# alex-petrenko/sample-factory

Hardware: AMD Instinct MI355X
Metric: env-steps/sec (whole node), 4096 envs, 84x84x4 obs (higher is better)
Workload: dtype f32

## Files before the change

### sample_factory_amd/csrc/sf_nn_img.h

```cpp
#pragma once

#ifndef SF_IMG_FLIP
#define SF_IMG_FLIP 1
#endif
#ifndef SF_IMG_PRIO
#define SF_IMG_PRIO 0
#endif
#ifndef SF_IMG_HALFSTEP
#define SF_IMG_HALFSTEP 1
#endif
template <int CIN, int H, int W, int KS, int ST, int TMF, int WSETS, int R>
struct ImgFwdGeom {
    static constexpr int OH = (H - KS) / ST + 1, OW = (W - KS) / ST + 1, OHW = R * OW;
    static constexpr int U = OH / R, HU = (R - 1) * ST + KS;
    static constexpr int K = KS * KS * CIN, KG = K / 16;
    static constexpr int C4 = CIN / 4, WQ = W / ST;
    static constexpr int PLANE_USED = ST * HU * WQ;
    static constexpr int PLANE = SF_IMG_FLIP ? (PLANE_USED + 15) / 16 * 16 : PLANE_USED;
    static constexpr int IMG_CH = C4 * PLANE;
    static constexpr int IMG_B = (IMG_CH * 16 + 1023) / 1024 * 1024;
    static constexpr int BROWS = WSETS * TMF * 16;
    static constexpr int RING = (2 * BROWS - 2) / OHW + 2;
    static_assert(CIN % 16 == 0 && W % ST == 0 && K % 16 == 0 && OH % R == 0, "geometry");
    static_assert(RING * IMG_B <= 160 * 1024, "LDS");
};

template <int CIN, int H, int W, int KS, int ST, int TMF, int WSETS, int R>
__global__ __launch_bounds__(256 * WSETS, 1) void k_fwd_img(const float *__restrict__ in, int64_t in_stride,
                                                    const float *__restrict__ wt, const float *__restrict__ bias,
                                                    float *__restrict__ out, int nsamples, int act) {
    typedef ImgFwdGeom<CIN, H, W, KS, ST, TMF, WSETS, R> G;
    constexpr int NW = 4 * WSETS, TB = TMF * WSETS;
    constexpr int OW = G::OW, OHW = G::OHW, K = G::K, KG = G::KG, WQ = G::WQ, PLANE = G::PLANE, RING = G::RING;
    constexpr int IMG_B = G::IMG_B, N = 64, U = G::U, HU = G::HU;
    __shared__ __attribute__((aligned(1024))) char ring[RING * IMG_B];
    const int tid = threadIdx.x, lane = tid & 63, wave = __builtin_amdgcn_readfirstlane(tid >> 6);
    const int col = lane & 15, kg = lane >> 4, n = (wave & 3) * 16 + col, wset = wave >> 2;
#if SF_IMG_PRIO
    if (__builtin_amdgcn_s_getreg((3 << 11) | (0 << 6) | 4) & 1u) __builtin_amdgcn_s_setprio(SF_IMG_PRIO);
#endif
    const int nunits = nsamples * U;
    const int64_t Mtot = (int64_t)nunits * OHW;
    const int total_frags = (int)((Mtot + 15) >> 4);
    const int per = (total_frags + (int)gridDim.x - 1) / (int)gridDim.x;
    const int f_beg = (int)blockIdx.x * per, f_end = min(total_frags, f_beg + per);
    if (f_beg >= f_end) return;
    f32x4 breg[KG];
#pragma unroll
    for (int g = 0; g < KG; ++g)
        breg[g] = *reinterpret_cast<const f32x4 *>(__builtin_assume_aligned(wt + (int64_t)n * K + 16 * g + 4 * kg, 16));
    const float bv = bias ? bias[n] : 0.f;

    constexpr int NDMA = IMG_B / 1024, NI = (NDMA + NW - 1) / NW;
    int srcoff[NI];
#pragma unroll
    for (int j = 0; j < NI; ++j) {
        int q = (wave + NW * j) * 64 + lane;
        q = q < G::IMG_CH ? q : 0;
        const int c = q / PLANE;
        int r0 = q - c * PLANE;
        r0 = r0 < G::PLANE_USED ? r0 : 0;
        const int pw = r0 / (HU * WQ), r1 = r0 - pw * (HU * WQ);
        const int ihl = r1 / WQ, iwq = r1 - ihl * WQ;
        const int ih = SF_IMG_FLIP ? HU - 1 - ihl : ihl;
        srcoff[j] = (ih * W + iwq * ST + pw) * CIN + c * 4;
    }
    auto load_image = [&](int s) {
        const int u = s < nunits ? s : nunits - 1, smp = u / U, strip = u - smp * U;
        const float *img = in + (int64_t)smp * in_stride + strip * (R * ST * W * CIN);
        char *dst = ring + (s % RING) * IMG_B;
#pragma unroll
        for (int j = 0; j < NI; ++j)
            if (wave + NW * j < NDMA) GLDS16(img + srcoff[j], dst + (wave + NW * j) * 1024);
    };
    const uint32_t M32 = (uint32_t)Mtot;
    auto last_sample = [&](int fb, int nf) {
        uint32_t m = (uint32_t)(fb + nf) * 16u - 1u;
        m = m < M32 ? m : M32 - 1u;
        return (int)(m / (uint32_t)OHW);
    };
    int loaded = (int)(((uint32_t)f_beg * 16u) / (uint32_t)OHW);
    {
        const int hi = last_sample(f_beg, min(TB, f_end - f_beg));
        for (; loaded <= hi; ++loaded) load_image(loaded);
    }
    f32x4 pend[TMF];
    int pend_fb = -1, pend_nf = 0;
    auto store_pend = [&]() {
        float *ob = out + ((int64_t)pend_fb * 16 + 4 * kg) * N + n;
        const int rows_left = (int)(M32 - ((uint32_t)pend_fb * 16u + 4u * (uint32_t)kg));
#pragma unroll
        for (int f = 0; f < TMF; ++f)
#pragma unroll
            for (int r = 0; r < 4; ++r)
                if (f < pend_nf && f * 16 + r < rows_left) ob[(f * 16 + r) * N] = pend[f][r];
    };
    for (int fb0 = f_beg; fb0 < f_end; fb0 += TB) {
        const int fb = fb0 + wset * TMF;
        const int nf = max(0, min(TMF, f_end - fb));
        asm volatile("s_waitcnt vmcnt(0)" ::: "memory");
        __syncthreads();
        if (fb0 + TB < f_end) {
            const int hi = last_sample(fb0 + TB, min(TB, f_end - fb0 - TB));
            for (; loaded <= hi; ++loaded) load_image(loaded);
        }
        if (pend_fb >= 0) store_pend();
        int base[TMF];
#pragma unroll
        for (int f = 0; f < TMF; ++f) {
            uint32_t m = (uint32_t)(nf > 0 ? fb + (f < nf ? f : 0) : fb0) * 16u + (uint32_t)col;
            m = m < M32 ? m : M32 - 1u;
            const uint32_t s = m / (uint32_t)OHW, p = m - s * (uint32_t)OHW, oh = p / (uint32_t)OW, ow = p - oh * (uint32_t)OW;
            const uint32_t prow = SF_IMG_FLIP ? ((uint32_t)(R - 1) - oh) * ST : oh * ST;
            base[f] = (int)((s % (uint32_t)RING) * (uint32_t)IMG_B + ((uint32_t)kg * PLANE + prow * WQ + ow) * 16u);
        }
        auto compute = [&](auto nfc) {
        constexpr int NF = decltype(nfc)::value;
        f32x4 acc[NF];
#pragma unroll
        for (int f = 0; f < NF; ++f) acc[f] = f32x4{0.f, 0.f, 0.f, 0.f};
        static_assert(KG % 2 == 0, "k-groups come in pairs");
        f32x4 a[2][2][NF];
        auto fetch = [&](int g, int slot) {
            const int tap = (16 * g) / CIN, cb = ((16 * g) % CIN) / 4, kh = tap / KS, kw = tap % KS;
            const int imm = (cb * PLANE + ((kw % ST) * HU + (SF_IMG_FLIP ? KS - 1 - kh : kh)) * WQ + kw / ST) * 16;
#pragma unroll
            for (int f = 0; f < NF; ++f)
                a[slot][g & 1][f] = *reinterpret_cast<const f32x4 *>(__builtin_assume_aligned(ring + base[f] + imm, 16));
        };
        auto mfmas = [&](int g, int slot) {
#pragma unroll
            for (int j = 0; j < 4; ++j)
#pragma unroll
                for (int f = 0; f < NF; ++f)
                    acc[f] = __builtin_amdgcn_mfma_f32_16x16x4f32(a[slot][g & 1][f][j], breg[g][j], acc[f], 0, 0, 0);
        };
        fetch(0, 0);
        fetch(1, 0);
#pragma unroll
        for (int gp = 0; gp < KG / 2; ++gp) {
            mfmas(2 * gp, gp & 1);
            __builtin_amdgcn_sched_barrier(0);
            if (gp + 1 < KG / 2) {
                fetch(2 * gp + 2, (gp + 1) & 1);
                fetch(2 * gp + 3, (gp + 1) & 1);
            }
            __builtin_amdgcn_sched_barrier(0);
            mfmas(2 * gp + 1, gp & 1);
            __builtin_amdgcn_sched_barrier(0);
        }
        auto park = [&](auto kc) {
            constexpr int KIND = decltype(kc)::value;
#pragma unroll
            for (int f = 0; f < NF; ++f)
#pragma unroll
                for (int r = 0; r < 4; ++r) pend[f][r] = act_fwd_c<KIND>(acc[f][r] + bv, act);
        };
        if (act == 1) park(std::integral_constant<int, 1>{});
        else park(std::integral_constant<int, -1>{});
        };
        if (SF_IMG_HALFSTEP && TMF == 2 && nf == 1) compute(std::integral_constant<int, 1>{});
        else compute(std::integral_constant<int, TMF>{});
        pend_fb = fb;
        pend_nf = nf;
    }
    if (pend_fb >= 0) store_pend();
}
```

### sample_factory_amd/csrc/sf_nn_glds.h

```cpp
#pragma once

#ifndef SF_GLDS_ABLATE
#define SF_GLDS_ABLATE 0
#endif
#define GLDS16(gsrc, ldst)                                                                       \
    __builtin_amdgcn_global_load_lds((const __attribute__((address_space(1))) void *)(gsrc),    \
                                     (__attribute__((address_space(3))) void *)(ldst), 16, 0, 0)

#define BARRIER_NOFENCE()                  \
    do {                                   \
        asm volatile("" ::: "memory");     \
        __builtin_amdgcn_s_barrier();      \
        asm volatile("" ::: "memory");     \
    } while (0)

template <int TM, int TN>
__device__ __forceinline__ void mma_chunk_rows(const float *__restrict__ As, const float *__restrict__ Bs, int arow0,
                                               int brow0, int lane, f32x16 (&acc)[TM][TN]) {
    const int r = lane & 31, h = lane >> 5, sw = (r >> 1) & 7;
    const float *ap = As + (arow0 + r) * 32, *bp = Bs + (brow0 + r) * 32;
#pragma unroll
    for (int c = 0; c < 4; ++c) {
        const int pos = (((2 * c + h) ^ sw) << 2);
        float4 a[TM], b[TN];
// ... 36 lines not shown
                    j == 0 ? b[c & 1][tn].x : j == 1 ? b[c & 1][tn].y : j == 2 ? b[c & 1][tn].z : b[c & 1][tn].w,
                    acc[tm][tn], 0, 0, 0);
    };
    fetch(0);
#pragma unroll
    for (int c = 0; c < 4; ++c) {
        mfmas(c, 0);
        mfmas(c, 1);
        __builtin_amdgcn_sched_barrier(0);
        mid(c);
        if (c + 1 < 4) fetch(c + 1);
        __builtin_amdgcn_sched_barrier(0);
        mfmas(c, 2);
        mfmas(c, 3);
    }
}

__device__ __forceinline__ void glds16_s(const void *ubase, uint32_t voff, uint32_t lds_byte_addr) {
    asm volatile("s_mov_b32 m0, %0\n\ts_nop 0\n\tglobal_load_lds_dwordx4 %1, %2"
                 :: "s"(lds_byte_addr), "v"(voff), "s"(ubase) : "memory", "m0");
}

template <int I, int N, typename F>
__device__ __forceinline__ void sf_static_for(F &&f) {
    if constexpr (I < N) {
        f(std::integral_constant<int, I>{});
        sf_static_for<I + 1, N>(f);
    }
}
template <int IMM>
__device__ __forceinline__ void glds16_si(const void *ubase, uint32_t voff, uint32_t lds_base) {
    asm volatile("s_add_u32 m0, %0, %3\n\ts_nop 0\n\tglobal_load_lds_dwordx4 %1, %2"
                 :: "s"(lds_base), "v"(voff), "s"(ubase), "n"(IMM) : "memory", "m0", "scc");
}

template <int TM, int TN, int OFF, typename F>
__device__ __forceinline__ void mma_chunk_ptrs_mid(const float *const (&ap)[4], const float *const (&bp)[4],
                                                   f32x16 (&acc)[TM][TN], F &&mid) {
    float4 a[2][TM], b[2][TN];
    auto fetch = [&](int c) {
#pragma unroll
        for (int i = 0; i < TM; ++i) a[c & 1][i] = *reinterpret_cast<const float4 *>(ap[c] + OFF + i * 32 * 32);
#pragma unroll
        for (int i = 0; i < TN; ++i) b[c & 1][i] = *reinterpret_cast<const float4 *>(bp[c] + OFF + i * 32 * 32);
    };
    auto mfmas = [&](int c, int j) {
#pragma unroll
        for (int tm = 0; tm < TM; ++tm)
#pragma unroll
            for (int tn = 0; tn < TN; ++tn)
                acc[tm][tn] = __builtin_amdgcn_mfma_f32_32x32x2f32(
                    j == 0 ? a[c & 1][tm].x : j == 1 ? a[c & 1][tm].y : j == 2 ? a[c & 1][tm].z : a[c & 1][tm].w,
                    j == 0 ? b[c & 1][tn].x : j == 1 ? b[c & 1][tn].y : j == 2 ? b[c & 1][tn].z : b[c & 1][tn].w,
                    acc[tm][tn], 0, 0, 0);
    };
    fetch(0);
#pragma unroll
    for (int c = 0; c < 4; ++c) {
        mfmas(c, 0);
        mfmas(c, 1);
        __builtin_amdgcn_sched_barrier(0);
        mid(c);
        if (c + 1 < 4) fetch(c + 1);
        __builtin_amdgcn_sched_barrier(0);
        mfmas(c, 2);
        mfmas(c, 3);
    }
}

template <int TM, int TN, int OFF, bool ZEROC = false>
__device__ __forceinline__ void mma_chunk_ptrs(const float *const (&ap)[4], const float *const (&bp)[4],
                                               f32x16 (&acc)[TM][TN]) {
#pragma unroll
    for (int c = 0; c < 4; ++c) {
        float4 a[TM], b[TN];
#pragma unroll
        for (int i = 0; i < TM; ++i) a[i] = *reinterpret_cast<const float4 *>(ap[c] + OFF + i * 32 * 32);
#pragma unroll
        for (int i = 0; i < TN; ++i) b[i] = *reinterpret_cast<const float4 *>(bp[c] + OFF + i * 32 * 32);
#pragma unroll
        for (int j = 0; j < 4; ++j)
#pragma unroll
            for (int tm = 0; tm < TM; ++tm)
#pragma unroll
                for (int tn = 0; tn < TN; ++tn) {
                    const f32x16 zero = {0.f, 0.f, 0.f, 0.f, 0.f, 0.f, 0.f, 0.f, 0.f, 0.f, 0.f, 0.f, 0.f, 0.f, 0.f, 0.f};
                    acc[tm][tn] = __builtin_amdgcn_mfma_f32_32x32x2f32(
                        j == 0 ? a[tm].x : j == 1 ? a[tm].y : j == 2 ? a[tm].z : a[tm].w,
                        j == 0 ? b[tn].x : j == 1 ? b[tn].y : j == 2 ? b[tn].z : b[tn].w,
                        (ZEROC && c == 0 && j == 0) ? zero : acc[tm][tn], 0, 0, 0);
                }
    }
}

#ifndef SF_FWD_FRAG_DB
#define SF_FWD_FRAG_DB 0
#endif
#ifndef SF_QUADROW_FRAG_DB
#define SF_QUADROW_FRAG_DB 2
#endif
template <int P> using HookPt = std::integral_constant<int, P>;
#ifndef SF_FRAG_DB_SINK
#define SF_FRAG_DB_SINK 16
#endif
template <int TM, int TN, int OFF, bool ZEROC = false, bool SPREAD = false, typename F>
__device__ __forceinline__ void mma_chunk_ptrs_db(const float *const (&ap)[4], const float *const (&bp)[4],
                                                  f32x16 (&acc)[TM][TN], F &&hook) {
    float4 a[2][TM], b[2][TN];
    auto fetch = [&](int c) {
#pragma unroll
        for (int i = 0; i < TM; ++i) a[c & 1][i] = *reinterpret_cast<const float4 *>(ap[c] + OFF + i * 32 * 32);
#pragma unroll
        for (int i = 0; i < TN; ++i) b[c & 1][i] = *reinterpret_cast<const float4 *>(bp[c] + OFF + i * 32 * 32);
    };
    auto mfmas = [&](int c, int j) {
#pragma unroll
        for (int tm = 0; tm < TM; ++tm)
#pragma unroll
            for (int tn = 0; tn < TN; ++tn) {
                const f32x16 zero = {0.f, 0.f, 0.f, 0.f, 0.f, 0.f, 0.f, 0.f, 0.f, 0.f, 0.f, 0.f, 0.f, 0.f, 0.f, 0.f};
                acc[tm][tn] = __builtin_amdgcn_mfma_f32_32x32x2f32(
                    j == 0 ? a[c & 1][tm].x : j == 1 ? a[c & 1][tm].y : j == 2 ? a[c & 1][tm].z : a[c & 1][tm].w,
                    j == 0 ? b[c & 1][tn].x : j == 1 ? b[c & 1][tn].y : j == 2 ? b[c & 1][tn].z : b[c & 1][tn].w,
                    (ZEROC && c == 0 && j == 0) ? zero : acc[tm][tn], 0, 0, 0);
            }
    };
    constexpr int PER = TM * TN;
    fetch(0);
    hook(HookPt<0>{});
#pragma unroll
    for (int c = 0; c < 4; ++c) {
        mfmas(c, 0);
        if (c + 1 < 4 || c == 0) {
            __builtin_amdgcn_sched_barrier(0);
            if (c == 0) hook(HookPt<1>{});
            if (c + 1 < 4) fetch(c + 1);
            __builtin_amdgcn_sched_barrier(0);
        } else if (SF_FRAG_DB_SINK == 3 * PER) __builtin_amdgcn_sched_barrier(0);
        mfmas(c, 1);
        if (c == 0 && SPREAD) {
            __builtin_amdgcn_sched_barrier(0);
            hook(HookPt<2>{});
            __builtin_amdgcn_sched_barrier(0);
        }
        if (c == 3 && SF_FRAG_DB_SINK == 2 * PER) __builtin_amdgcn_sched_barrier(0);
        mfmas(c, 2);
        if (c == 3 && SF_FRAG_DB_SINK == PER) __builtin_amdgcn_sched_barrier(0);
        mfmas(c, 3);
        if (c == 0) hook(HookPt<3>{});
        if (c == 3 && SF_FRAG_DB_SINK == 0) __builtin_amdgcn_sched_barrier(0);
    }
}

#ifndef SF_PIX_INCR
#define SF_PIX_INCR 1
#endif
#ifndef SF_PIX_LDSIMM
#define SF_PIX_LDSIMM 1
#endif
#ifndef SF_QUADROW_ROT
#define SF_QUADROW_ROT 0
#endif
#ifndef SF_QUADROW_PREP
#define SF_QUADROW_PREP 1
#endif
#ifndef SF_DGRAD_PIX_ZL_LITE
#define SF_DGRAD_PIX_ZL_LITE 1
#endif
template <int TM, int TN, int STAGE_F>
__device__ __forceinline__ void mma_chunk_stage(const float *const (&ap)[4], const float *const (&bp)[4], int stage,
                                                f32x16 (&acc)[TM][TN]) {
    if (stage == 0) mma_chunk_ptrs<TM, TN, 0>(ap, bp, acc);
    else mma_chunk_ptrs<TM, TN, STAGE_F>(ap, bp, acc);
}

template <int BM, int BN, int WM, int WN, int NS, bool ZL, bool PERSIST = false, bool DYNLDS = false>
__device__ __forceinline__ void fwd_glds_body(ConvG g, const float *__restrict__ in, int64_t in_stride,
                                              const float *__restrict__ wt, const float *__restrict__ bias,
                                              float *__restrict__ out, int64_t Mtot, int k_per_split,
                                              float *__restrict__ partial, const float *__restrict__ dmask,
                                              int dmask_on, int rx, int ry, int rtot, int tap_perm, int bx_shift = 0) {
    constexpr int TM = BM / WM / 32, TN = BN / WN / 32;
    constexpr int AI = BM / 32, BI = BN / 32;
    constexpr int STAGE = (BM + BN) * 32;
    static_assert(WM * WN == 4 && TM >= 1 && TN >= 1 && (NS == 2 || NS == 3), "4 waves per block");
    __shared__ __attribute__((aligned(1024))) float lds_static[DYNLDS ? 1 : NS * STAGE];
    extern __shared__ __attribute__((aligned(1024))) float lds_dynamic[];
    float *const lds = DYNLDS ? lds_dynamic : lds_static;
    const int tid = threadIdx.x, lane = tid & 63, wave = __builtin_amdgcn_readfirstlane(tid >> 6);
    const int wm = wave / WN, wn = wave % WN;
    const int ptiles = PERSIST ? (int)((Mtot + BM - 1) / BM) : 1;
    for (int ptile = PERSIST ? (int)blockIdx.x : 0; ptile < ptiles; ptile += PERSIST ? (int)gridDim.x : 1) {
    int bx = PERSIST ? ptile : (int)blockIdx.x + bx_shift, by = blockIdx.y, bz = blockIdx.z;
    if (rtot > 0) {
        const int per = (rtot + 7) >> 3, L = (int)(blockIdx.x & 7u) * per + (int)(blockIdx.x >> 3);
        if (L >= rtot) return;
        by = L % ry;
        const int t = L / ry;
        bx = t % rx;
        bz = t / rx;
    }
    const int64_t m0 = (int64_t)bx * BM;
    const int n0 = by * BN;
    const int N = g.Cout, K = g.K;
    const int kbeg = bz * k_per_split, kend = min(K, kbeg + k_per_split);

    const int lrow = lane >> 3, lpos = lane & 7;
    const float *asrc[AI], *bsrc[BI];
#pragma unroll
    for (int i = 0; i < AI; ++i) {
        const int row = (i * 4 + wave) * 8 + lrow;
        int64_t m = m0 + row;
        m = m < Mtot ? m : Mtot - 1;
        const uint32_t smp = fdiv((uint32_t)m, g.dOHOW), pix = (uint32_t)m - smp * (uint32_t)(g.OH * g.OW);
        asrc[i] = in + (int64_t)smp * in_stride + patch_origin<false>(g, pix) + ((lpos ^ ((row >> 1) & 7)) << 2);
    }
#pragma unroll
    for (int i = 0; i < BI; ++i) {
        const int row = (i * 4 + wave) * 8 + lrow;
        int n = n0 + row;
        n = n < N ? n : N - 1;
        bsrc[i] = wt + (int64_t)n * K + ((lpos ^ ((row >> 1) & 7)) << 2);
    }
    f32x16 acc[TM][TN];
#pragma unroll
    for (int a_ = 0; a_ < TM; ++a_)
#pragma unroll
        for (int b_ = 0; b_ < TN; ++b_)
#pragma unroll
            for (int r_ = 0; r_ < 16; ++r_) acc[a_][b_][r_] = 0.f;

    auto issue = [&](int k0, int stage) {
        const uint32_t tap = fdiv((uint32_t)k0, g.dCin), c0 = (uint32_t)k0 - tap * (uint32_t)g.Cin;
        const uint32_t kh = fdiv(tap, g.dKW), kw = tap - kh * (uint32_t)g.KW;
        const int aoff = (int)((kh * (uint32_t)g.W + kw) * (uint32_t)g.Cin + c0);
        float *sa = lds + stage * STAGE, *sb = sa + BM * 32;
#pragma unroll
        for (int i = 0; i < AI; ++i) GLDS16(asrc[i] + aoff, sa + (i * 4 + wave) * 256);
#pragma unroll
        for (int i = 0; i < BI; ++i) GLDS16(bsrc[i] + k0, sb + (i * 4 + wave) * 256);
    };
    static_assert(NS == 2, "two LDS stages");
    const bool tapperm = tap_perm && g.KH == 4 && g.KW == 4 && g.S == 2 && g.Cin == 32 && kbeg == 0 && kend == K;
    auto kord = [&](int k0) {
        if (!tapperm) return k0;
        const int p = k0 >> 5, grp = p >> 2, e = p & 3;
        const int kh = ((grp >> 1) & 1) + 2 * (e >> 1), kw = (grp & 1) + 2 * (e & 1);
        return (kh * 4 + kw) << 5;
    };
    int stage = 0, k0 = kbeg;
    constexpr bool MASK_PRE = ZL && TM * TN == 4;
    float mpre[MASK_PRE ? TM : 1][MASK_PRE ? TN : 1][16];
    bool mask_pre = false;
    auto prefetch_mask = [&]() {
        if constexpr (MASK_PRE) {
            if (dmask_on && dmask && g.relu == 1 && m0 + BM <= Mtot && n0 + BN <= N) {
                const float *mk = dmask + (m0 + wm * TM * 32) * N + (n0 + wn * TN * 32);
                const uint32_t vo = (uint32_t)(4 * (lane >> 5)) * (uint32_t)N + (uint32_t)(lane & 31);
#pragma unroll
                for (int tm = 0; tm < TM; ++tm)
#pragma unroll
                    for (int tn = 0; tn < TN; ++tn)
#pragma unroll
                        for (int r = 0; r < 16; ++r)
                            mpre[tm][tn][r] = (mk + (int64_t)(tm * 32 + (r & 3) + 8 * (r >> 2)) * N + tn * 32)[vo];
                mask_pre = true;
            }
        }
    };
    if constexpr (ZL) {

        uint32_t avoff[AI], bvoff[BI];
#pragma unroll
        for (int i = 0; i < AI; ++i) avoff[i] = (uint32_t)((asrc[i] - in) * (int64_t)sizeof(float));
#pragma unroll
        for (int i = 0; i < BI; ++i) bvoff[i] = (uint32_t)((bsrc[i] - wt) * (int64_t)sizeof(float));
        const uint32_t lds0 = (uint32_t)(uintptr_t)(__attribute__((address_space(3))) float *)lds;
        const int r = lane & 31, h = lane >> 5, sw = (r >> 1) & 7;
        const float *apl[4], *bpl[4];
#pragma unroll
        for (int c = 0; c < 4; ++c) {
            const int pos = (((2 * c + h) ^ sw) << 2);
            apl[c] = lds + (wm * TM * 32 + r) * 32 + pos;
            bpl[c] = lds + BM * 32 + (wn * TN * 32 + r) * 32 + pos;
        }
        auto chunk_off = [&](int kn) {
            const uint32_t tap = fdiv((uint32_t)kn, g.dCin), c0 = (uint32_t)kn - tap * (uint32_t)g.Cin;
            const uint32_t kh = fdiv(tap, g.dKW), kw = tap - kh * (uint32_t)g.KW;
            return (int)((kh * (uint32_t)g.W + kw) * (uint32_t)g.Cin + c0);
        };
        auto dma = [&](int q, const float *abase, const float *bbase, int st) {
            if (q < AI) glds16_s(abase, avoff[q < AI ? q : 0], lds0 + (uint32_t)((st * STAGE + (q * 4 + wave) * 256) * 4));
            else glds16_s(bbase, bvoff[q >= AI ? q - AI : 0], lds0 + (uint32_t)((st * STAGE + BM * 32 + ((q - AI) * 4 + wave) * 256) * 4));
        };
        {
            const int kf = kord(kbeg);
            const float *ab = in + chunk_off(kf), *bb = wt + kf;
#pragma unroll
            for (int q = 0; q < AI + BI; ++q) dma(q, ab, bb, 0);
        }
        auto step = [&](auto stc, bool prefetch) {
            constexpr int ST = decltype(stc)::value;
            asm volatile("s_waitcnt vmcnt(0)" ::: "memory");
            BARRIER_NOFENCE();
            const int kn = prefetch ? kord(k0 + 32) : 0;
            const float *ab = in + chunk_off(kn), *bb = wt + kn;
            if (!prefetch) prefetch_mask();
            if constexpr (TM * TN <= 2) {
                mma_chunk_ptrs_mid<TM, TN, ST * STAGE>(apl, bpl, acc, [&](int c) {
                    constexpr int TOT = AI + BI, PER = (TOT + 2) / 3;
                    if (prefetch) {
#pragma unroll
                        for (int q = 0; q < TOT; ++q)
                            if (q / PER == c) dma(q, ab, bb, ST ^ 1);
                    }
                });
            } else {
                auto burst = [&](int qlo, int qhi) {
                    if (prefetch) {
#pragma unroll
                        for (int q = 0; q < AI + BI; ++q)
                            if (q >= qlo && q < qhi) dma(q, ab, bb, ST ^ 1);
                    }
                };
                if constexpr (SF_FWD_FRAG_DB >= 2) {
                    mma_chunk_ptrs_db<TM, TN, ST * STAGE, false, SF_FWD_FRAG_DB == 3>(apl, bpl, acc, [&](auto pt) {
                        constexpr int P = decltype(pt)::value, HALF = (AI + BI) / 2;
                        if constexpr (SF_FWD_FRAG_DB == 2) {
                            if constexpr (P == 0) burst(0, AI + BI);
                        } else {
                            if constexpr (P == 1) burst(0, HALF);
                            if constexpr (P == 2) burst(HALF, AI + BI);
                        }
                    });
                } else {
                    burst(0, AI + BI);
                    if constexpr (SF_FWD_FRAG_DB == 1) mma_chunk_ptrs_db<TM, TN, ST * STAGE>(apl, bpl, acc, [](auto) {});
                    else mma_chunk_ptrs<TM, TN, ST * STAGE>(apl, bpl, acc);
                }
            }
            k0 += 32;
        };
        while (k0 + 64 < kend) {
            step(std::integral_constant<int, 0>{}, true);
            step(std::integral_constant<int, 1>{}, true);
        }
        if (k0 + 32 < kend) {
            step(std::integral_constant<int, 0>{}, true);
            step(std::integral_constant<int, 1>{}, false);
        } else {
            step(std::integral_constant<int, 0>{}, false);
        }
    } else {
    issue(kord(kbeg), 0);
    if constexpr (TM * TN <= 2) {
        for (; k0 + 32 < ((SF_GLDS_ABLATE & 8) ? kbeg + 64 : kend); k0 += 32, stage ^= 1) {
            if (!(SF_GLDS_ABLATE & 2)) {
            asm volatile("s_waitcnt vmcnt(0)" ::: "memory");
            BARRIER_NOFENCE();
            }
            const int kn = kord(k0 + 32);
            const uint32_t tap = fdiv((uint32_t)kn, g.dCin), c0 = (uint32_t)kn - tap * (uint32_t)g.Cin;
            const uint32_t kh = fdiv(tap, g.dKW), kw = tap - kh * (uint32_t)g.KW;
            const int aoff = (int)((kh * (uint32_t)g.W + kw) * (uint32_t)g.Cin + c0);
            float *na = lds + (stage ^ 1) * STAGE, *nb = na + BM * 32;
            const float *sa = lds + stage * STAGE;
            mma_chunk_rows_mid<TM, TN>(sa, sa + BM * 32, wm * TM * 32, wn * TN * 32, lane, acc, [&](int c) {
                constexpr int TOT = AI + BI, PER = (TOT + 2) / 3;
#pragma unroll
                for (int q = 0; q < TOT; ++q) {
                    if (q / PER != c || (SF_GLDS_ABLATE & 1)) continue;
                    if (q < AI) GLDS16(asrc[q < AI ? q : 0] + aoff, na + (q * 4 + wave) * 256);
                    else GLDS16(bsrc[q >= AI ? q - AI : 0] + kn, nb + ((q - AI) * 4 + wave) * 256);
                }
            });
        }
    } else {
        for (; k0 + 32 < kend; k0 += 32, stage ^= 1) {
            asm volatile("s_waitcnt vmcnt(0)" ::: "memory");
            BARRIER_NOFENCE();
            issue(k0 + 32, stage ^ 1);
            const float *sa = lds + stage * STAGE;
            mma_chunk_rows<TM, TN>(sa, sa + BM * 32, wm * TM * 32, wn * TN * 32, lane, acc);
        }
    }
    asm volatile("s_waitcnt vmcnt(0)" ::: "memory");
    BARRIER_NOFENCE();
    {
        const float *sa = lds + stage * STAGE;
        mma_chunk_rows<TM, TN>(sa, sa + BM * 32, wm * TM * 32, wn * TN * 32, lane, acc);
    }
    }
    float *ob = (partial ? partial + (int64_t)bz * Mtot * N : out) + (m0 + wm * TM * 32) * N + (n0 + wn * TN * 32);
    const int rows_left = (int)min((int64_t)(TM * 32), Mtot - m0 - wm * TM * 32) - 4 * (lane >> 5);
    const int cols_left = N - (n0 + wn * TN * 32) - (lane & 31);
    const uint32_t voff = (uint32_t)(4 * (lane >> 5)) * (uint32_t)N + (uint32_t)(lane & 31);
    const bool full = m0 + BM <= Mtot && n0 + BN <= N;
    if (dmask_on) {
        const float *mk = dmask ? dmask + (m0 + wm * TM * 32) * N + (n0 + wn * TN * 32) : nullptr;
        if (!dmask) {
            if (full) store_dgrad_tile<TM, TN, 0, true>(acc, ob, mk, voff, N, rows_left, cols_left, 0);
            else store_dgrad_tile<TM, TN, 0, false>(acc, ob, mk, voff, N, rows_left, cols_left, 0);
        } else if (MASK_PRE && mask_pre) {
#pragma unroll
            for (int tn = 0; tn < TN; ++tn)
#pragma unroll
                for (int tm = 0; tm < TM; ++tm)
#pragma unroll
                    for (int r = 0; r < 16; ++r) {
                        const int rr = tm * 32 + (r & 3) + 8 * (r >> 2);
                        (ob + (int64_t)rr * N + tn * 32)[voff] = act_bwd_mul<1>(acc[tm][tn][r], mpre[MASK_PRE ? tm : 0][MASK_PRE ? tn : 0][r], 1);
                    }
        } else if (g.relu == 1) {
            if (full) store_dgrad_tile<TM, TN, 1, true>(acc, ob, mk, voff, N, rows_left, cols_left, 1);
            else store_dgrad_tile<TM, TN, 1, false>(acc, ob, mk, voff, N, rows_left, cols_left, 1);
        } else {
            store_dgrad_tile<TM, TN, -1, false>(acc, ob, mk, voff, N, rows_left, cols_left, g.relu);
        }
    } else if (partial) {
        if (full) store_fwd_tile<TM, TN, 0, true>(acc, ob, voff, N, rows_left, cols_left, nullptr, lane & 31, 0);
        else store_fwd_tile<TM, TN, 0, false>(acc, ob, voff, N, rows_left, cols_left, nullptr, lane & 31, 0);
    } else if (g.relu == 1) {
        if (full) store_fwd_tile<TM, TN, 1, true>(acc, ob, voff, N, rows_left, cols_left, bias ? bias + n0 + wn * TN * 32 : nullptr, lane & 31, 1);
        else store_fwd_tile<TM, TN, 1, false>(acc, ob, voff, N, rows_left, cols_left, bias ? bias + n0 + wn * TN * 32 : nullptr, lane & 31, 1);
    } else {
        store_fwd_tile<TM, TN, -1, false>(acc, ob, voff, N, rows_left, cols_left, bias ? bias + n0 + wn * TN * 32 : nullptr, lane & 31, g.relu);
    }
    if (PERSIST) BARRIER_NOFENCE();
    }
}

template <int BM, int BN, int WM, int WN, int NS>
__global__ __launch_bounds__(256) void k_fwd_glds(ConvG g, const float *__restrict__ in, int64_t in_stride,
                                                  const float *__restrict__ wt, const float *__restrict__ bias,
                                                  float *__restrict__ out, int64_t Mtot, int k_per_split,
                                                  float *__restrict__ partial, const float *__restrict__ dmask,
                                                  int dmask_on, int rx = 0, int ry = 0, int rtot = 0, int tap_perm = 0) {
    fwd_glds_body<BM, BN, WM, WN, NS, false>(g, in, in_stride, wt, bias, out, Mtot, k_per_split, partial, dmask, dmask_on, rx,
                                             ry, rtot, tap_perm);
}
template <int BM, int BN, int WM, int WN>
__global__ __launch_bounds__(256, 2) void k_fwd_glds_zp(ConvG g, const float *__restrict__ in, int64_t in_stride,
                                                       const float *__restrict__ wt, const float *__restrict__ bias,
                                                       float *__restrict__ out, int64_t Mtot, int k_per_split) {
    fwd_glds_body<BM, BN, WM, WN, 2, true, true>(g, in, in_stride, wt, bias, out, Mtot, k_per_split, nullptr, nullptr, 0, 0, 0, 0, 0);
}
template <int BM, int BN, int WM, int WN>
__global__ __launch_bounds__(256, 2) void k_fwd_glds_zt(ConvG g, const float *__restrict__ in, int64_t in_stride,
                                                       const float *__restrict__ wt, const float *__restrict__ bias,
                                                       float *__restrict__ out, int64_t Mtot, int k_per_split, int main_tiles,
                                                       int tap_perm) {
    if ((int)blockIdx.x < main_tiles)
        fwd_glds_body<BM, BN, WM, WN, 2, true, false, true>(g, in, in_stride, wt, bias, out, Mtot, k_per_split, nullptr, nullptr, 0,
                                                            0, 0, 0, tap_perm);
    else
        fwd_glds_body<BM / 2, BN, WM, WN, 2, true, false, true>(g, in, in_stride, wt, bias, out, Mtot, k_per_split, nullptr,
                                                                nullptr, 0, 0, 0, 0, tap_perm, main_tiles);
}
template <int BM, int BN, int WM, int WN>
__global__ __launch_bounds__(256, 2) void k_fwd_glds_z(ConvG g, const float *__restrict__ in, int64_t in_stride,
                                                    const float *__restrict__ wt, const float *__restrict__ bias,
                                                    float *__restrict__ out, int64_t Mtot, int k_per_split,
                                                    float *__restrict__ partial, const float *__restrict__ dmask,
                                                    int dmask_on, int rx = 0, int ry = 0, int rtot = 0, int tap_perm = 0) {
    fwd_glds_body<BM, BN, WM, WN, 2, true>(g, in, in_stride, wt, bias, out, Mtot, k_per_split, partial, dmask, dmask_on, rx, ry,
                                           rtot, tap_perm);
}

template <int BM, int BN, int WM, int WN>
__global__ __launch_bounds__(256) void k_fwd_glds2(const float *__restrict__ a1, int64_t lda1, const float *__restrict__ w1t,
                                                   const float *__restrict__ bias1, int K1, const float *__restrict__ a2,
                                                   int64_t lda2, const float *__restrict__ w2t,
                                                   const float *__restrict__ bias2, int K2, float *__restrict__ out,
                                                   int64_t Mtot, int N, int gru_H) {
    constexpr int TM = BM / WM / 32, TN = BN / WN / 32;
    constexpr int AI = BM / 32, BI = BN / 32;
    constexpr int STAGE = (BM + BN) * 32;
    static_assert(WM * WN == 4 && TM >= 1 && TN >= 1, "4 waves per block");
    __shared__ __attribute__((aligned(1024))) float lds[2 * STAGE];
    const int tid = threadIdx.x, lane = tid & 63, wave = __builtin_amdgcn_readfirstlane(tid >> 6);
    const int wm = wave / WN, wn = wave % WN;
    const int64_t m0 = (int64_t)blockIdx.x * BM;
    const int n0 = blockIdx.y * BN;
    const bool use1 = gru_H == 0 || n0 < 3 * gru_H, use2 = gru_H == 0 || n0 < 2 * gru_H || n0 >= 3 * gru_H;
    const int row2_off = (gru_H > 0 && n0 >= 3 * gru_H) ? -gru_H : 0;
    const int kbeg = use1 ? 0 : K1, K = use2 ? K1 + K2 : K1;
    const int lrow = lane >> 3, lpos = lane & 7;
    const float *as1[AI], *as2[AI], *bs1[BI], *bs2[BI];
#pragma unroll
    for (int i = 0; i < AI; ++i) {
        const int row = (i * 4 + wave) * 8 + lrow;
        int64_t m = m0 + row;
        m = m < Mtot ? m : Mtot - 1;
        const int sw = (lpos ^ ((row >> 1) & 7)) << 2;
        as1[i] = a1 + m * lda1 + sw;
        as2[i] = a2 + m * lda2 + sw - K1;
    }
#pragma unroll
    for (int i = 0; i < BI; ++i) {
        const int row = (i * 4 + wave) * 8 + lrow;
        int n = n0 + row;
        n = n < N ? n : N - 1;
        const int sw = (lpos ^ ((row >> 1) & 7)) << 2;
        bs1[i] = w1t + (int64_t)(use1 ? n : 0) * K1 + sw;
        bs2[i] = w2t + (int64_t)(use2 ? n + row2_off : 0) * K2 + sw - K1;
    }
    f32x16 acc[TM][TN];
#pragma unroll
    for (int a_ = 0; a_ < TM; ++a_)
#pragma unroll
        for (int b_ = 0; b_ < TN; ++b_)
#pragma unroll
            for (int r_ = 0; r_ < 16; ++r_) acc[a_][b_][r_] = 0.f;
    auto issue = [&](int k0, int stage) {
        float *sa = lds + stage * STAGE, *sb = sa + BM * 32;
        const bool first = k0 < K1;
#pragma unroll
        for (int i = 0; i < AI; ++i) GLDS16((first ? as1[i] : as2[i]) + k0, sa + (i * 4 + wave) * 256);
#pragma unroll
        for (int i = 0; i < BI; ++i) GLDS16((first ? bs1[i] : bs2[i]) + k0, sb + (i * 4 + wave) * 256);
    };
    issue(kbeg, 0);
    int stage = 0, k0 = kbeg;
    for (; k0 + 32 < K; k0 += 32, stage ^= 1) {
        asm volatile("s_waitcnt vmcnt(0)" ::: "memory");
        BARRIER_NOFENCE();
        issue(k0 + 32, stage ^ 1);
        const float *sa = lds + stage * STAGE;
        mma_chunk_rows<TM, TN>(sa, sa + BM * 32, wm * TM * 32, wn * TN * 32, lane, acc);
    }
    asm volatile("s_waitcnt vmcnt(0)" ::: "memory");
    BARRIER_NOFENCE();
    {
        const float *sa = lds + stage * STAGE;
        mma_chunk_rows<TM, TN>(sa, sa + BM * 32, wm * TM * 32, wn * TN * 32, lane, acc);
    }
    const int lcol = lane & 31;
#pragma unroll
    for (int tn = 0; tn < TN; ++tn) {
        const int col = n0 + wn * TN * 32 + tn * 32 + lcol;
        if (col >= N) continue;
        const float b1 = (bias1 && use1) ? bias1[col] : 0.f, b2 = (bias2 && use2) ? bias2[col + row2_off] : 0.f;
#pragma unroll
        for (int tm = 0; tm < TM; ++tm)
#pragma unroll
            for (int r = 0; r < 16; ++r) {
                const int64_t row = m0 + wm * TM * 32 + tm * 32 + FRAG_ROW(r, lane);
                if (row < Mtot) out[row * N + col] = (acc[tm][tn][r] + b1) + b2;
            }
    }
}

__global__ __launch_bounds__(256) void k_transpose(const float *__restrict__ w, float *__restrict__ wt, int K, int N) {
    __shared__ float t[32][33];
    const int k0 = blockIdx.x * 32, n0 = blockIdx.y * 32, tx = threadIdx.x & 31, ty = threadIdx.x >> 5;
#pragma unroll
    for (int i = 0; i < 32; i += 8) {
        const int k = k0 + ty + i, n = n0 + tx;
        t[ty + i][tx] = (k < K && n < N) ? w[(int64_t)k * N + n] : 0.f;
    }
    __syncthreads();
#pragma unroll
    for (int i = 0; i < 32; i += 8) {
        const int n = n0 + ty + i, k = k0 + tx;
// ... 1205 lines not shown
```

Baseline: 2.112 million.

## Interleave image DMA into MFMA k-loop and stagger blocks on odd slots

Issues the global-to-LDS image loads in small pieces between MFMA k-group pairs instead of in a burst before compute. Replaces per-step division-based address computation with incremental pixel/slot advancement, and adds a fast unguarded store path for full tiles. Blocks on odd hardware slots (read via s_getreg) take a one-fragment half step first so co-resident blocks are out of phase, replacing the setprio experiment. The aim is to hide load latency and smooth memory contention, at the cost of more complex control flow and address bookkeeping.

```diff
diff --git a/sample_factory_amd/csrc/sf_nn_img.h b/sample_factory_amd/csrc/sf_nn_img.h
--- a/sample_factory_amd/csrc/sf_nn_img.h
+++ b/sample_factory_amd/csrc/sf_nn_img.h
@@ -2,9 +2,6 @@
 
 #ifndef SF_IMG_FLIP
 #define SF_IMG_FLIP 1
-#endif
-#ifndef SF_IMG_PRIO
-#define SF_IMG_PRIO 0
 #endif
 #ifndef SF_IMG_HALFSTEP
 #define SF_IMG_HALFSTEP 1
@@ -25,6 +22,11 @@
     static_assert(RING * IMG_B <= 160 * 1024, "LDS");
 };
 
+constexpr int img_dma_gap(int gp, int npairs, int ngap) {
+    for (int i = 0; i < ngap; ++i)
+        if (((i + 1) * npairs) / (ngap + 1) == gp) return i;
+    return -1;
+}
 template <int CIN, int H, int W, int KS, int ST, int TMF, int WSETS, int R>
 __global__ __launch_bounds__(256 * WSETS, 1) void k_fwd_img(const float *__restrict__ in, int64_t in_stride,
                                                     const float *__restrict__ wt, const float *__restrict__ bias,
@@ -34,11 +36,11 @@
     constexpr int OW = G::OW, OHW = G::OHW, K = G::K, KG = G::KG, WQ = G::WQ, PLANE = G::PLANE, RING = G::RING;
     constexpr int IMG_B = G::IMG_B, N = 64, U = G::U, HU = G::HU;
     __shared__ __attribute__((aligned(1024))) char ring[RING * IMG_B];
+    __shared__ int odd_slot_s;
     const int tid = threadIdx.x, lane = tid & 63, wave = __builtin_amdgcn_readfirstlane(tid >> 6);
     const int col = lane & 15, kg = lane >> 4, n = (wave & 3) * 16 + col, wset = wave >> 2;
-#if SF_IMG_PRIO
-    if (__builtin_amdgcn_s_getreg((3 << 11) | (0 << 6) | 4) & 1u) __builtin_amdgcn_s_setprio(SF_IMG_PRIO);
-#endif
+    constexpr bool STAGGER = SF_IMG_HALFSTEP && TMF == 2 && WSETS == 1;
+    if (STAGGER && tid == 0) odd_slot_s = (int)(__builtin_amdgcn_s_getreg((3 << 11) | (0 << 6) | 4) & 1u);
     const int nunits = nsamples * U;
     const int64_t Mtot = (int64_t)nunits * OHW;
     const int total_frags = (int)((Mtot + 15) >> 4);
@@ -52,7 +54,7 @@
     const float bv = bias ? bias[n] : 0.f;
 
     constexpr int NDMA = IMG_B / 1024, NI = (NDMA + NW - 1) / NW;
-    int srcoff[NI];
+    uint32_t srcoff[NI];
 #pragma unroll
     for (int j = 0; j < NI; ++j) {
         int q = (wave + NW * j) * 64 + lane;
@@ -63,59 +65,100 @@
         const int pw = r0 / (HU * WQ), r1 = r0 - pw * (HU * WQ);
         const int ihl = r1 / WQ, iwq = r1 - ihl * WQ;
         const int ih = SF_IMG_FLIP ? HU - 1 - ihl : ihl;
-        srcoff[j] = (ih * W + iwq * ST + pw) * CIN + c * 4;
-    }
-    auto load_image = [&](int s) {
-        const int u = s < nunits ? s : nunits - 1, smp = u / U, strip = u - smp * U;
-        const float *img = in + (int64_t)smp * in_stride + strip * (R * ST * W * CIN);
-        char *dst = ring + (s % RING) * IMG_B;
-#pragma unroll
-        for (int j = 0; j < NI; ++j)
-            if (wave + NW * j < NDMA) GLDS16(img + srcoff[j], dst + (wave + NW * j) * 1024);
-    };
+        srcoff[j] = (uint32_t)((ih * W + iwq * ST + pw) * CIN + c * 4) * 4u;
+    }
     const uint32_t M32 = (uint32_t)Mtot;
-    auto last_sample = [&](int fb, int nf) {
+    auto last_unit = [&](int fb, int nf) {
         uint32_t m = (uint32_t)(fb + nf) * 16u - 1u;
         m = m < M32 ? m : M32 - 1u;
         return (int)(m / (uint32_t)OHW);
     };
+    const uint32_t lds0 = (uint32_t)(uintptr_t)(__attribute__((address_space(3))) char *)ring;
     int loaded = (int)(((uint32_t)f_beg * 16u) / (uint32_t)OHW);
+    int ld_strip = loaded % U, ld_slot = loaded % RING;
+    const float *ld_img = in + (int64_t)(loaded / U) * in_stride + ld_strip * (R * ST * W * CIN);
+    auto loader_next = [&]() {
+        ++loaded;
+        ld_slot = ld_slot + 1 == RING ? 0 : ld_slot + 1;
+        ld_img += R * ST * W * CIN;
+        if (++ld_strip == U) {
+            ld_strip = 0;
+            ld_img += in_stride - (int64_t)U * (R * ST * W * CIN);
+        }
+    };
+    auto piece = [&](auto qc, int nnew) {
+        constexpr int Q = decltype(qc)::value, I = Q / NI, J = Q % NI;
+        if (I < nnew) {
+            if (NDMA % NW == 0 || wave + NW * J < NDMA)
+                glds16_si<NW * J * 1024>(ld_img, srcoff[J], lds0 + (uint32_t)ld_slot * IMG_B + (uint32_t)wave * 1024u);
+            if (J == NI - 1) loader_next();
+        }
+    };
+    constexpr int MAXNEW = (G::BROWS + OHW - 1) / OHW, NPIECE = MAXNEW * NI;
+    constexpr int PPG = 2, NGAP = (NPIECE + PPG - 1) / PPG;
+    static_assert(NGAP < KG / 2, "more DMA gaps than k-group pairs");
+
+    constexpr uint32_t DIV_M = 65536u / OW + 1u;
+    static_assert((uint32_t)(OHW - 1) * DIV_M < (1u << 24) && ((OW - 65536 % OW) * (OHW - 1)) < 65536, "pixel / OW by multiplication");
+    constexpr int LIN0 = SF_IMG_FLIP ? (R - 1) * ST * WQ : 0, LIN1 = SF_IMG_FLIP ? -(ST * WQ + OW) : ST * WQ - OW;
+    const int kgoff = (kg * PLANE + LIN0) * 16;
+    uint32_t pix[TMF], soff[TMF];
+    int base[TMF];
+    auto address = [&](int f) {
+        const uint32_t oh = __umul24(pix[f], DIV_M) >> 16;
+        return (int)soff[f] + kgoff + ((int)pix[f] + (int)oh * LIN1) * 16;
+    };
+    auto advance = [&](auto rowsc) {
+        constexpr int ROWS = decltype(rowsc)::value, QU = ROWS / OHW, REM = ROWS % OHW;
+#pragma unroll
+        for (int f = 0; f < TMF; ++f) {
+            pix[f] += REM;
+            const bool wrap = pix[f] >= (uint32_t)OHW;
+            pix[f] = wrap ? pix[f] - OHW : pix[f];
+            soff[f] += wrap ? (QU + 1) * IMG_B : QU * IMG_B;
+#pragma unroll
+            for (int i = 0; i < (QU + 1 + RING - 1) / RING; ++i) soff[f] = soff[f] >= RING * IMG_B ? soff[f] - RING * IMG_B : soff[f];
+        }
+    };
+#pragma unroll
+    for (int f = 0; f < TMF; ++f) {
+        const uint32_t m = (uint32_t)(f_beg + wset * TMF + f) * 16u + (uint32_t)col, s = m / (uint32_t)OHW;
+        pix[f] = m - s * (uint32_t)OHW;
+        soff[f] = (s % (uint32_t)RING) * (uint32_t)IMG_B;
+        base[f] = address(f);
+    }
+    int odd_slot = 0;
+    if (STAGGER) {
+        __syncthreads();
+        odd_slot = __builtin_amdgcn_readfirstlane(odd_slot_s);
+    }
+    int adv = (STAGGER && odd_slot) ? 1 : TB;
     {
-        const int hi = last_sample(f_beg, min(TB, f_end - f_beg));
-        for (; loaded <= hi; ++loaded) load_image(loaded);
+        const int hi = last_unit(f_beg, min(adv, f_end - f_beg));
+        while (loaded <= hi) sf_static_for<0, NI>([&](auto jc) { piece(jc, 1); });
     }
     f32x4 pend[TMF];
     int pend_fb = -1, pend_nf = 0;
+    const uint32_t lane_out = (uint32_t)(4 * kg * N + n);
     auto store_pend = [&]() {
-        float *ob = out + ((int64_t)pend_fb * 16 + 4 * kg) * N + n;
-        const int rows_left = (int)(M32 - ((uint32_t)pend_fb * 16u + 4u * (uint32_t)kg));
-#pragma unroll
-        for (int f = 0; f < TMF; ++f)
-#pragma unroll
-            for (int r = 0; r < 4; ++r)
-                if (f < pend_nf && f * 16 + r < rows_left) ob[(f * 16 + r) * N] = pend[f][r];
-    };
-    for (int fb0 = f_beg; fb0 < f_end; fb0 += TB) {
-        const int fb = fb0 + wset * TMF;
-        const int nf = max(0, min(TMF, f_end - fb));
-        asm volatile("s_waitcnt vmcnt(0)" ::: "memory");
-        __syncthreads();
-        if (fb0 + TB < f_end) {
-            const int hi = last_sample(fb0 + TB, min(TB, f_end - fb0 - TB));
-            for (; loaded <= hi; ++loaded) load_image(loaded);
-        }
-        if (pend_fb >= 0) store_pend();
-        int base[TMF];
-#pragma unroll
-        for (int f = 0; f < TMF; ++f) {
-            uint32_t m = (uint32_t)(nf > 0 ? fb + (f < nf ? f : 0) : fb0) * 16u + (uint32_t)col;
-            m = m < M32 ? m : M32 - 1u;
-            const uint32_t s = m / (uint32_t)OHW, p = m - s * (uint32_t)OHW, oh = p / (uint32_t)OW, ow = p - oh * (uint32_t)OW;
-            const uint32_t prow = SF_IMG_FLIP ? ((uint32_t)(R - 1) - oh) * ST : oh * ST;
-            base[f] = (int)((s % (uint32_t)RING) * (uint32_t)IMG_B + ((uint32_t)kg * PLANE + prow * WQ + ow) * 16u);
-        }
-        auto compute = [&](auto nfc) {
-        constexpr int NF = decltype(nfc)::value;
+        if (pend_nf == TMF && (uint32_t)(pend_fb + TMF) * 16u <= M32) {
+            float *ob = out + (int64_t)pend_fb * (16 * N);
+#pragma unroll
+            for (int f = 0; f < TMF; ++f)
+#pragma unroll
+                for (int r = 0; r < 4; ++r) ob[lane_out + (uint32_t)((f * 16 + r) * N)] = pend[f][r];
+        } else {
+            float *ob = out + ((int64_t)pend_fb * 16 + 4 * kg) * N + n;
+            const int rows_left = (int)(M32 - ((uint32_t)pend_fb * 16u + 4u * (uint32_t)kg));
+#pragma unroll
+            for (int f = 0; f < TMF; ++f)
+#pragma unroll
+                for (int r = 0; r < 4; ++r)
+                    if (f < pend_nf && f * 16 + r < rows_left) ob[(f * 16 + r) * N] = pend[f][r];
+        }
+    };
+    auto step = [&](auto nfc, auto advc, int fb, int nf, int nnew) {
+        constexpr int NF = decltype(nfc)::value, ADV = decltype(advc)::value;
         f32x4 acc[NF];
 #pragma unroll
         for (int f = 0; f < NF; ++f) acc[f] = f32x4{0.f, 0.f, 0.f, 0.f};
@@ -137,18 +180,28 @@
         };
         fetch(0, 0);
         fetch(1, 0);
-#pragma unroll
-        for (int gp = 0; gp < KG / 2; ++gp) {
+        __builtin_amdgcn_sched_barrier(0);
+        if (pend_fb >= 0) store_pend();
+        int nbase[TMF];
+        advance(std::integral_constant<int, ADV * 16>{});
+#pragma unroll
+        for (int f = 0; f < TMF; ++f) nbase[f] = address(f);
+        sf_static_for<0, KG / 2>([&](auto gpc) {
+            constexpr int gp = decltype(gpc)::value;
             mfmas(2 * gp, gp & 1);
             __builtin_amdgcn_sched_barrier(0);
             if (gp + 1 < KG / 2) {
                 fetch(2 * gp + 2, (gp + 1) & 1);
                 fetch(2 * gp + 3, (gp + 1) & 1);
             }
+            if constexpr (img_dma_gap(gp, KG / 2, NGAP) >= 0) {
+                constexpr int Q0 = img_dma_gap(gp, KG / 2, NGAP) * PPG, Q1 = Q0 + PPG < NPIECE ? Q0 + PPG : NPIECE;
+                sf_static_for<Q0, Q1>([&](auto qc) { piece(qc, nnew); });
+            }
             __builtin_amdgcn_sched_barrier(0);
             mfmas(2 * gp + 1, gp & 1);
             __builtin_amdgcn_sched_barrier(0);
-        }
+        });
         auto park = [&](auto kc) {
             constexpr int KIND = decltype(kc)::value;
 #pragma unroll
@@ -158,11 +211,23 @@
         };
         if (act == 1) park(std::integral_constant<int, 1>{});
         else park(std::integral_constant<int, -1>{});
-        };
-        if (SF_IMG_HALFSTEP && TMF == 2 && nf == 1) compute(std::integral_constant<int, 1>{});
-        else compute(std::integral_constant<int, TMF>{});
+#pragma unroll
+        for (int f = 0; f < TMF; ++f) base[f] = nbase[f];
         pend_fb = fb;
         pend_nf = nf;
+    };
+    for (int fb0 = f_beg; fb0 < f_end;) {
+        const int fb = fb0 + wset * (adv == TB ? TMF : 0);
+        const int nf = max(0, min(adv == TB ? TMF : 1, f_end - fb));
+        const int next = fb0 + adv;
+        const int nnew = next < f_end ? last_unit(next, min(TB, f_end - next)) - loaded + 1 : 0;
+        asm volatile("s_waitcnt vmcnt(0)" ::: "memory");
+        __syncthreads();
+        if (STAGGER && adv == 1) step(std::integral_constant<int, 1>{}, std::integral_constant<int, 1>{}, fb, nf, nnew);
+        else if (SF_IMG_HALFSTEP && TMF == 2 && nf == 1) step(std::integral_constant<int, 1>{}, std::integral_constant<int, TB>{}, fb, nf, nnew);
+        else step(std::integral_constant<int, TMF>{}, std::integral_constant<int, TB>{}, fb, nf, nnew);
+        fb0 = next;
+        adv = TB;
     }
     if (pend_fb >= 0) store_pend();
 }
```

After: 2.119 million, median of 6. No clear change (+0.3%).

## Stage dgrad ReLU mask through LDS via async global-to-LDS loads

Applied to the files above, without the earlier changes.

In the ZL dgrad path with 2x2 warp tiles, the ReLU mask used to be prefetched into 64 registers per lane. It is now DMA'd into the free LDS stage with global_load_lds, in two halves. The first half is issued during the last K step and the second after a barrier in the epilogue, and the store loop then reads the mask values from LDS. This is meant to cut register pressure and use wide 16-byte coalesced loads. In exchange it adds an extra barrier, vmcnt waits and LDS reads in the epilogue, and it needs N%4==0 and a 16-byte-aligned mask.

```diff
diff --git a/sample_factory_amd/csrc/sf_nn_glds.h b/sample_factory_amd/csrc/sf_nn_glds.h
--- a/sample_factory_amd/csrc/sf_nn_glds.h
+++ b/sample_factory_amd/csrc/sf_nn_glds.h
@@ -212,6 +212,9 @@
     }
 }
 
+#ifndef SF_FC_MASK_LDS
+#define SF_FC_MASK_LDS 1
+#endif
 #ifndef SF_PIX_INCR
 #define SF_PIX_INCR 1
 #endif
@@ -310,10 +313,33 @@
     };
     int stage = 0, k0 = kbeg;
     constexpr bool MASK_PRE = ZL && TM * TN == 4;
-    float mpre[MASK_PRE ? TM : 1][MASK_PRE ? TN : 1][16];
+    constexpr bool MASK_LDS = MASK_PRE && SF_FC_MASK_LDS != 0;
+    static_assert(!MASK_LDS || STAGE / 4 >= TM * TN * 2 * 256, "a wave's quarter of a stage holds half of its mask pieces");
+    float mpre[MASK_PRE && !MASK_LDS ? TM : 1][MASK_PRE && !MASK_LDS ? TN : 1][MASK_PRE && !MASK_LDS ? 16 : 1];
     bool mask_pre = false;
-    auto prefetch_mask = [&]() {
-        if constexpr (MASK_PRE) {
+    int mask_st = 0;
+    auto stage_mask = [&](int half, int st) {
+        if constexpr (MASK_LDS) {
+            const float *mk = dmask + (m0 + wm * TM * 32) * N + (n0 + wn * TN * 32);
+            const uint32_t lds0 = (uint32_t)(uintptr_t)(__attribute__((address_space(3))) float *)lds;
+            const uint32_t vo = ((uint32_t)((lane >> 4) + 4 * ((lane >> 3) & 1)) * (uint32_t)N + (uint32_t)(4 * (lane & 7))) * 4u;
+            const uint32_t dst = lds0 + (uint32_t)((st * STAGE + wave * 2048) * 4);
+            sf_static_for<0, 8>([&](auto qc) {
+                constexpr int Q = decltype(qc)::value;
+                const int blk = 2 * half + (Q >> 2), tm = blk % TM, tn = blk / TM;
+                glds16_si<Q * 1024>(mk + (int64_t)(tm * 32 + 8 * (Q & 3)) * N + tn * 32, vo, dst);
+            });
+        }
+    };
+    auto prefetch_mask = [&](int st) {
+        if constexpr (MASK_LDS) {
+            if (dmask_on && dmask && g.relu == 1 && m0 + BM <= Mtot && n0 + BN <= N && (N & 3) == 0 &&
+                ((uintptr_t)dmask & 15) == 0) {
+                stage_mask(0, st ^ 1);
+                mask_st = st;
+                mask_pre = true;
+            }
+        } else if constexpr (MASK_PRE) {
             if (dmask_on && dmask && g.relu == 1 && m0 + BM <= Mtot && n0 + BN <= N) {
                 const float *mk = dmask + (m0 + wm * TM * 32) * N + (n0 + wn * TN * 32);
                 const uint32_t vo = (uint32_t)(4 * (lane >> 5)) * (uint32_t)N + (uint32_t)(lane & 31);
@@ -365,7 +391,7 @@
             BARRIER_NOFENCE();
             const int kn = prefetch ? kord(k0 + 32) : 0;
             const float *ab = in + chunk_off(kn), *bb = wt + kn;
-            if (!prefetch) prefetch_mask();
+            if (!prefetch) prefetch_mask(ST);
             if constexpr (TM * TN <= 2) {
                 mma_chunk_ptrs_mid<TM, TN, ST * STAGE>(apl, bpl, acc, [&](int c) {
                     constexpr int TOT = AI + BI, PER = (TOT + 2) / 3;
@@ -461,7 +487,31 @@
         if (!dmask) {
             if (full) store_dgrad_tile<TM, TN, 0, true>(acc, ob, mk, voff, N, rows_left, cols_left, 0);
             else store_dgrad_tile<TM, TN, 0, false>(acc, ob, mk, voff, N, rows_left, cols_left, 0);
-        } else if (MASK_PRE && mask_pre) {
+        } else if (MASK_LDS && mask_pre) {
+            typedef const __attribute__((address_space(3))) float *lds_cptr;
+            uint32_t ma0 = (uint32_t)(uintptr_t)(lds_cptr)(lds + (mask_st ^ 1) * STAGE + wave * 2048 + lane);
+            uint32_t ma1 = (uint32_t)(uintptr_t)(lds_cptr)(lds + mask_st * STAGE + wave * 2048 + lane);
+            asm volatile("s_waitcnt lgkmcnt(0)" : "+v"(ma0), "+v"(ma1) :: "memory");
+            lds_cptr ml = (lds_cptr)(uintptr_t)ma0;
+            BARRIER_NOFENCE();
+            stage_mask(1, mask_st);
+            asm volatile("s_waitcnt vmcnt(8)" ::: "memory");
+#pragma unroll
+            for (int blk = 0; blk < TM * TN; ++blk) {
+                const int tm = blk % TM, tn = blk / TM;
+                if (blk == 2) {
+                    if constexpr (SF_FC_MASK_LDS == 2) asm volatile("s_waitcnt vmcnt(32)" ::: "memory");
+                    else asm volatile("s_waitcnt vmcnt(0)" ::: "memory");
+                    ml = (lds_cptr)(uintptr_t)ma1;
+                }
+#pragma unroll
+                for (int r = 0; r < 16; ++r) {
+                    const int rr = tm * 32 + (r & 3) + 8 * (r >> 2);
+                    const float y = ml[((blk & 1) * 4 + (r >> 2)) * 256 + (r & 3) * 64];
+                    (ob + (int64_t)rr * N + tn * 32)[voff] = act_bwd_mul<1>(acc[tm][tn][r], y, 1);
+                }
+            }
+        } else if (MASK_PRE && !MASK_LDS && mask_pre) {
 #pragma unroll
             for (int tn = 0; tn < TN; ++tn)
 #pragma unroll
@@ -469,7 +519,7 @@
 #pragma unroll
                     for (int r = 0; r < 16; ++r) {
                         const int rr = tm * 32 + (r & 3) + 8 * (r >> 2);
-                        (ob + (int64_t)rr * N + tn * 32)[voff] = act_bwd_mul<1>(acc[tm][tn][r], mpre[MASK_PRE ? tm : 0][MASK_PRE ? tn : 0][r], 1);
+                        (ob + (int64_t)rr * N + tn * 32)[voff] = act_bwd_mul<1>(acc[tm][tn][r], mpre[MASK_PRE && !MASK_LDS ? tm : 0][MASK_PRE && !MASK_LDS ? tn : 0][MASK_PRE && !MASK_LDS ? r : 0], 1);
                     }
         } else if (g.relu == 1) {
             if (full) store_dgrad_tile<TM, TN, 1, true>(acc, ob, mk, voff, N, rows_left, cols_left, 1);
```

Measured after the change: 2.123 million before, 2.125 million after, median of 2. Within noise of the previous version (+0.1%).
